# JARVIS-MoCap/JARVIS-HybridNet

Hardware: AMD Instinct MI355X
Metric: multi-view frames/s (12cam 1280x1024, 23kpt, 64^3 grid) (higher is better)
Workload: dtype f32; 1 GPU; BASELINE configs[2]: HybridNet 12-camera 1280x1024, 23 kpts, 64^3 grid, small/small; cameras=12, joints=23, grid=64, streams=3, parallelism=single GPU, 3 time batches in flight on 3 HIP streams, hipgraph=False

## Files before the change

### include/jarvis_hip.h

```cpp
#ifndef JARVIS_HIP_H
#define JARVIS_HIP_H
#include <stdint.h>

#ifdef __cplusplus
extern "C" {
#endif

#define JH_ABI_VERSION 4

const char* jh_last_error(void);
int jh_abi_version(void);

#define JH_PRECISION_DEFAULT (-1)
#define JH_PRECISION_F32 0
#define JH_PRECISION_BF16X3 1
#define JH_PRECISION_BF16X3_WIDE 2
int jh_set_precision(int mode);
int jh_get_precision(void);

typedef struct jh_params jh_params;
int jh_params_create(jh_params** out);
int jh_params_set(jh_params* p, const char* key, const float* host, int64_t numel);
void jh_params_destroy(jh_params* p);

typedef struct jh_efftrack jh_efftrack;
int jh_efftrack_create(const jh_params* p, const char* prefix, int model_size, int joints, int n,
                       int h, int w, int want_res1, jh_efftrack** out);
int jh_efftrack_forward(jh_efftrack* net, const float* x_dev, float* res1_dev, float* res2_dev,
                        void* stream);
int64_t jh_efftrack_launches(const jh_efftrack* net);
void jh_efftrack_destroy(jh_efftrack* net);

typedef struct jh_v2v jh_v2v;
int jh_v2v_create(const jh_params* p, const char* prefix, int joints, int t, int g, jh_v2v** out);
int jh_v2v_forward(jh_v2v* net, const float* x_dev, float* y_dev, void* stream);
void jh_v2v_destroy(jh_v2v* net);
int jh_v2v_fold(int joints, int t, int g, int* folded);

int64_t jh_reproject_workspace_bytes(int cams, int joints, int hs, int grid_size);
int jh_reproject_forward(const float* heatmaps_padded_dev, int cams, int joints, int hs,
                         const int32_t* center3d_dev, const int32_t* center_hm_dev,
                         const float* cam_dev, const float* intr_dev, const float* dist_dev,
                         int grid_size, float grid_spacing, float* vol_dev, int32_t* idx_dev,
                         void* workspace_dev, int64_t workspace_bytes, void* stream);

int64_t jh_softargmax_workspace_bytes(int t, int joints, int gh);
int jh_softargmax(const float* v2v_out_dev, int t, int joints, int gh, float grid_spacing,
                  float roi_cube_size, const int32_t* center3d_dev, float* heatmap_final_dev,
                  float* points_dev, float* conf_dev, void* workspace_dev, int64_t workspace_bytes,
                  void* stream);

int jh_reproject_point(const float* points_dev, int npoints, int cams, const float* cam_dev,
                       const float* intr_dev, const float* dist_dev, float* uv_dev, void* stream);
int64_t jh_reconstruct_workspace_bytes(int cams);
int jh_reconstruct_point(const float* points2d_dev, const float* maxvals_dev, int cams,
                         const float* cam_dev, const float* intr_dev, const float* dist_dev,
                         float* point3d_dev, void* workspace_dev, int64_t workspace_bytes,
                         void* stream);

typedef struct jh_predictor jh_predictor;
typedef struct {
  int32_t num_cameras, num_joints;
  int32_t center_size;
  int32_t bbox;
  float roi_cube_size;
  float grid_spacing;
  int32_t center_model, kp_model;
  int32_t img_h, img_w;
  int32_t time_batch;
  int32_t time_batch_3d;
  int32_t cam_lo, cam_n;
  float mean[3], std[3];
  int32_t precision;
} jh_predictor_config;

int jh_predictor_create(const jh_params* center_params, const jh_params* hybrid_params,
                        const jh_predictor_config* cfg, jh_predictor** out);
void jh_predictor_destroy(jh_predictor* pr);
int64_t jh_predictor_launches(const jh_predictor* pr);
int64_t jh_predictor_device_bytes(const jh_predictor* pr);
int jh_predictor_precision(const jh_predictor* pr);

int jh_predictor_set_calibration(jh_predictor* pr, const float* cam_dev, const float* intr_dev,
                                 const float* dist_dev, void* stream);
int jh_predictor_set_calibration_frames(jh_predictor* pr, const float* cam_dev ,
                                        const float* intr_dev , const float* dist_dev ,
                                        void* stream);

int jh_predictor_set_centers(jh_predictor* pr, const float* centers_dev , void* stream);

// ... 195 lines not shown
```

### jarvis-hybridnet_amd/_native.py

```python
import ctypes
import math
import os
from typing import NamedTuple

import torch

_HERE = os.path.dirname(os.path.abspath(__file__))
LIB_PATH = os.environ.get("JH_LIBRARY_PATH") or os.path.join(_HERE, "libjarvis_hip.so")
_lib = None

c_void_p, c_int, c_float, c_int64 = ctypes.c_void_p, ctypes.c_int, ctypes.c_float, ctypes.c_int64
c_char_p = ctypes.c_char_p


class PredictorConfig(ctypes.Structure):
    _fields_ = [("num_cameras", ctypes.c_int32), ("num_joints", ctypes.c_int32),
                ("center_size", ctypes.c_int32), ("bbox", ctypes.c_int32),
                ("roi_cube_size", c_float), ("grid_spacing", c_float),
                ("center_model", ctypes.c_int32), ("kp_model", ctypes.c_int32),
                ("img_h", ctypes.c_int32), ("img_w", ctypes.c_int32),
                ("time_batch", ctypes.c_int32), ("time_batch_3d", ctypes.c_int32),
                ("cam_lo", ctypes.c_int32),
                ("cam_n", ctypes.c_int32), ("mean", c_float * 3), ("std", c_float * 3),
                ("precision", ctypes.c_int32)]
# ... 13 lines not shown
    _fields_ = [("image_stride", ctypes.c_int64), ("offset", ctypes.c_int64), ("pitch", ctypes.c_int64),
                ("pattern", ctypes.c_int32), ("reserved", ctypes.c_int32)]


assert ctypes.sizeof(SensorSurfaceStruct) == 32

class OpOperand(ctypes.Structure):
    _fields_ = [("in_sums_host", c_void_p), ("in_act", ctypes.c_int32), ("latency_class", ctypes.c_int32),
                ("want_stats", ctypes.c_int32), ("se_c", ctypes.c_int32), ("se_s", ctypes.c_int32),
                ("se_inv_hw", c_float), ("se_wr_host", c_void_p), ("se_br_host", c_void_p),
                ("se_we_host", c_void_p), ("se_be_host", c_void_p), ("se_pool_host", c_void_p)]


assert ctypes.sizeof(OpOperand) == 72

class SubjectsParamsStruct(ctypes.Structure):
    _fields_ = [("max_subjects", ctypes.c_int32), ("max_peaks", ctypes.c_int32), ("nms_radius", ctypes.c_int32),
                ("min_views", ctypes.c_int32), ("min_peak", c_float), ("max_error_px", c_float)]


assert ctypes.sizeof(SubjectsParamsStruct) == 24

ABI_VERSION = 4
assert ctypes.sizeof(PredictorConfig) == 84

_WORKSPACES = {}


def workspace(nbytes, device):
    key = (str(device), torch.cuda.current_stream(device).cuda_stream)
    bufs = _WORKSPACES.setdefault(key, [])
    if not bufs or bufs[-1].numel() < nbytes:
        bufs.append(torch.empty((max(int(nbytes), 256),), dtype=torch.uint8, device=device))
    return bufs[-1]


_SIGS = {
    "jh_last_error": (c_char_p, []),
    "jh_abi_version": (c_int, []),
    "jh_set_precision": (c_int, [c_int]),
    "jh_get_precision": (c_int, []),
    "jh_params_create": (c_int, [ctypes.POINTER(c_void_p)]),
    "jh_params_set": (c_int, [c_void_p, c_char_p, c_void_p, c_int64]),
    "jh_params_destroy": (None, [c_void_p]),
    "jh_efftrack_create": (c_int, [c_void_p, c_char_p, c_int, c_int, c_int, c_int, c_int, c_int,
                                   ctypes.POINTER(c_void_p)]),
    "jh_efftrack_forward": (c_int, [c_void_p, c_void_p, c_void_p, c_void_p, c_void_p]),
    "jh_efftrack_launches": (c_int64, [c_void_p]),
    "jh_efftrack_destroy": (None, [c_void_p]),
    "jh_v2v_create": (c_int, [c_void_p, c_char_p, c_int, c_int, c_int, ctypes.POINTER(c_void_p)]),
    "jh_v2v_forward": (c_int, [c_void_p, c_void_p, c_void_p, c_void_p]),
    "jh_v2v_destroy": (None, [c_void_p]),
    "jh_v2v_fold": (c_int, [c_int, c_int, c_int, ctypes.POINTER(c_int)]),
    "jh_reproject_workspace_bytes": (c_int64, [c_int, c_int, c_int, c_int]),
    "jh_reproject_forward": (c_int, [c_void_p, c_int, c_int, c_int, c_void_p, c_void_p, c_void_p,
                                     c_void_p, c_void_p, c_int, c_float, c_void_p, c_void_p,
                                     c_void_p, c_int64, c_void_p]),
    "jh_softargmax_workspace_bytes": (c_int64, [c_int, c_int, c_int]),
    "jh_softargmax": (c_int, [c_void_p, c_int, c_int, c_int, c_float, c_float, c_void_p, c_void_p,
                              c_void_p, c_void_p, c_void_p, c_int64, c_void_p]),
    "jh_softargmax_spread_workspace_bytes": (c_int64, [c_int, c_int, c_int]),
    "jh_softargmax_spread": (c_int, [c_void_p, c_int, c_int, c_int, c_float, c_float, c_void_p, c_void_p,
                                     c_void_p, c_void_p, c_void_p, c_void_p, c_void_p, c_void_p, c_int64, c_void_p]),
    "jh_predictor_set_spread": (c_int, [c_void_p, c_int]),
    "jh_predictor_get_spread": (c_int, [c_void_p, c_void_p, c_void_p, c_void_p, c_void_p]),
    "jh_predictor_debug_v2v": (c_int, [c_void_p, c_void_p, c_void_p]),
    "jh_reproject_point": (c_int, [c_void_p, c_int, c_int, c_void_p, c_void_p, c_void_p, c_void_p,
                                   c_void_p]),
    "jh_reconstruct_workspace_bytes": (c_int64, [c_int]),
    "jh_reconstruct_point": (c_int, [c_void_p, c_void_p, c_int, c_void_p, c_void_p, c_void_p,
                                     c_void_p, c_void_p, c_int64, c_void_p]),
    "jh_predictor_create": (c_int, [c_void_p, c_void_p, ctypes.POINTER(PredictorConfig),
                                    ctypes.POINTER(c_void_p)]),
    "jh_predictor_destroy": (None, [c_void_p]),
    "jh_predictor_set_graph_replay": (c_int, [c_void_p, c_int]),
    "jh_predictor_graph_replay": (c_int, [c_void_p]),
    "jh_predictor_launches": (c_int64, [c_void_p]),
    "jh_predictor_device_bytes": (c_int64, [c_void_p]),
    "jh_predictor_precision": (c_int, [c_void_p]),
    "jh_predictor_set_calibration": (c_int, [c_void_p, c_void_p, c_void_p, c_void_p, c_void_p]),
    "jh_predictor_set_calibration_frames": (c_int, [c_void_p, c_void_p, c_void_p, c_void_p, c_void_p]),
    "jh_predictor_set_centers": (c_int, [c_void_p, c_void_p, c_void_p]),
    "jh_predictor_stage_center": (c_int, [c_void_p, c_void_p, c_void_p, c_void_p]),
    "jh_predictor_stage_keypoints": (c_int, [c_void_p, c_void_p, c_void_p, c_void_p, c_void_p]),
    "jh_predictor_stage_3d": (c_int, [c_void_p, c_void_p, c_int, c_void_p, c_void_p, c_void_p,
                                      c_void_p]),
    "jh_predictor_stage_keypoints_gathered": (c_int, [c_void_p, c_void_p, c_int, c_void_p, c_int, c_void_p,
                                                      c_void_p]),
    "jh_predictor_stage_3d_blocks": (c_int, [c_void_p, c_void_p, c_int, c_int, c_int, c_int, c_void_p,
                                             c_void_p, c_void_p, c_void_p]),
    "jh_profile_begin": (c_int, []),
    "jh_profile_end": (c_int, [ctypes.POINTER(c_int)]),
    "jh_profile_get": (c_int, [c_int, c_char_p, c_int, ctypes.POINTER(ctypes.c_double),
                               ctypes.POINTER(ctypes.c_double), ctypes.POINTER(ctypes.c_double)]),
    "jh_predictor_forward": (c_int, [c_void_p, c_void_p, c_void_p, c_void_p, c_void_p, c_void_p]),
    "jh_predictor_stage_center_u8": (c_int, [c_void_p, c_void_p, c_void_p, c_void_p]),
    "jh_predictor_stage_keypoints_u8": (c_int, [c_void_p, c_void_p, c_void_p, c_void_p, c_void_p]),
    "jh_predictor_forward_u8": (c_int, [c_void_p, c_void_p, c_void_p, c_void_p, c_void_p, c_void_p]),
    "jh_predictor_forward_yuv": (c_int, [c_void_p, c_void_p, c_int, c_void_p, c_void_p, c_void_p, c_void_p]),
    "jh_yuv_surface_check": (c_int, [ctypes.POINTER(YuvSurfaceStruct), c_int, c_int]),
    "jh_predictor_forward_surface": (c_int, [c_void_p, c_void_p, ctypes.POINTER(YuvSurfaceStruct), c_void_p, c_void_p,
                                             c_void_p, c_void_p, c_void_p]),
    "jh_predictor2d_forward_surface": (c_int, [c_void_p, c_void_p, ctypes.POINTER(YuvSurfaceStruct), c_void_p,
                                               c_void_p, c_void_p, c_void_p]),
    "jh_op_yuv_surface_to_bgr": (c_int, [c_void_p, ctypes.POINTER(YuvSurfaceStruct), c_int, c_int, c_int, c_void_p,
                                         c_void_p]),
# ... 404 lines not shown
```

### jarvis-hybridnet_amd/csrc/api.hip

```cpp
#include <cstring>
#include <memory>
#include "../../include/jarvis_hip.h"
#include <cstdlib>
#include "nets.h"
#include "bifpn_node.h"
#include "views2d.h"
#include "subjects.h"

namespace jh {
static thread_local std::string g_err;
void set_error(const std::string& msg) { g_err = msg; }
}

using namespace jh;

struct jh_params { ParamMap map; };
struct jh_efftrack { EffTrackPlan plan; };
struct jh_v2v { V2VPlan plan; };

namespace {

struct Scratch {
  std::vector<void*> ptrs;
  ~Scratch() { for (void* p : ptrs) (void)hipFree(p); }
// ... 126 lines not shown
  return 0;
}
int jh_get_precision(void) { return precision_mode(); }

int jh_params_create(jh_params** out) {
  *out = new jh_params();
  return 0;
}
int jh_params_set(jh_params* p, const char* key, const float* host, int64_t numel) {
  JH_REQUIRE(p && key && host && numel >= 0, "bad argument");
  p->map[key] = std::vector<float>(host, host + numel);
  return 0;
}
void jh_params_destroy(jh_params* p) { delete p; }

int jh_efftrack_create(const jh_params* p, const char* prefix, int model_size, int joints, int n,
                       int h, int w, int want_res1, jh_efftrack** out) {
  JH_REQUIRE(p && out, "bad argument");
  std::unique_ptr<jh_efftrack> net(new jh_efftrack());
  if (net->plan.build(p->map, prefix ? prefix : "", model_size, joints, n, h, w, want_res1 != 0)) return 1;
  *out = net.release();
  return 0;
}
int jh_efftrack_forward(jh_efftrack* net, const float* x_dev, float* res1_dev, float* res2_dev,
                        void* stream) {
  hipStream_t s = static_cast<hipStream_t>(stream);
  JH_REQUIRE(net && x_dev && res2_dev, "bad argument");
  JH_REQUIRE(!res1_dev || net->plan.res1.p, "res1 requested from a network created with want_res1 = 0");
  if (launch_to_channel_last(x_dev, net->plan.input, s)) return 1;
  if (net->plan.run(s)) return 1;
  if (res1_dev && launch_from_channel_last(net->plan.res1, res1_dev, s)) return 1;
  return launch_from_channel_last(net->plan.heat, res2_dev, s);
}
int64_t jh_efftrack_launches(const jh_efftrack* net) { return (int64_t)net->plan.launches(); }
void jh_efftrack_destroy(jh_efftrack* net) { delete net; }

int jh_v2v_create(const jh_params* p, const char* prefix, int joints, int t, int g, jh_v2v** out) {
  JH_REQUIRE(p && out, "bad argument");
  std::unique_ptr<jh_v2v> net(new jh_v2v());
  if (net->plan.build(p->map, prefix ? prefix : "", joints, t, g)) return 1;
  *out = net.release();
  return 0;
}
int jh_v2v_forward(jh_v2v* net, const float* x_dev, float* y_dev, void* stream) {
  hipStream_t s = static_cast<hipStream_t>(stream);
  if (launch_to_channel_last(x_dev, net->plan.input, s)) return 1;
  if (net->plan.run(s)) return 1;
  return launch_from_channel_last(net->plan.output, y_dev, s);
}
void jh_v2v_destroy(jh_v2v* net) { delete net; }
int jh_v2v_fold(int joints, int t, int g, int* folded) {
  JH_REQUIRE(joints >= 1 && t >= 1 && g >= 4 && g % 4 == 0 && folded, "jh_v2v_fold: bad argument");
  *folded = v2v_fold_applies(joints, g) ? 1 : 0;
  return 0;
}

int64_t jh_reproject_workspace_bytes(int cams, int joints, int hs, int grid_size) {
  Carver c(nullptr, 0);
  ReproWs w;
  return (int64_t)carve_reproject(c, cams, joints, hs, grid_size, &w);
}

int jh_reproject_forward(const float* heatmaps_padded_dev, int cams, int joints, int hs,
                         const int32_t* center3d_dev, const int32_t* center_hm_dev,
                         const float* cam_dev, const float* intr_dev, const float* dist_dev,
                         int grid_size, float grid_spacing, float* vol_dev, int32_t* idx_dev,
                         void* workspace_dev, int64_t workspace_bytes, void* stream) {
  hipStream_t s = static_cast<hipStream_t>(stream);
  JH_REQUIRE(workspace_dev && workspace_bytes >= 0, "workspace (see jh_reproject_workspace_bytes)");
  JH_REQUIRE(grid_size > 0 && grid_size % 2 == 0, "grid size must be even");
  Carver c(workspace_dev, (size_t)workspace_bytes);
  ReproWs w;
  carve_reproject(c, cams, joints, hs, grid_size, &w);
  JH_REQUIRE(c.fits(), "workspace smaller than jh_reproject_workspace_bytes()");
  if (launch_to_channel_last(heatmaps_padded_dev, w.heat, s)) return 1;
  if (launch_reproject(Calib{cam_dev, intr_dev, dist_dev, 0}, center3d_dev, center_hm_dev, w.heat.p, w.coarse,
                       w.vol.p, idx_dev, 1, cams, grid_size, grid_spacing, hs, w.heat.Cp,
                       1, 0, nullptr, s)) return 1;
  return launch_from_channel_last(w.vol, vol_dev, s);
}

int64_t jh_softargmax_workspace_bytes(int t, int joints, int gh) {
  Carver c(nullptr, 0);
  SoftWs w;
  return (int64_t)carve_softargmax(c, t, joints, gh, &w);
}

int jh_softargmax(const float* v2v_out_dev, int t, int joints, int gh, float grid_spacing,
                  float roi_cube_size, const int32_t* center3d_dev, float* heatmap_final_dev,
                  float* points_dev, float* conf_dev, void* workspace_dev, int64_t workspace_bytes,
                  void* stream) {
  hipStream_t s = static_cast<hipStream_t>(stream);
  JH_REQUIRE(workspace_dev && workspace_bytes >= 0, "workspace (see jh_softargmax_workspace_bytes)");
  Carver c(workspace_dev, (size_t)workspace_bytes);
  SoftWs w;
  carve_softargmax(c, t, joints, gh, &w);
  JH_REQUIRE(c.fits(), "workspace smaller than jh_softargmax_workspace_bytes()");
  if (launch_to_channel_last(v2v_out_dev, w.x, s)) return 1;
  return launch_softargmax(w.x.p, center3d_dev, w.partial, w.pmax, points_dev, conf_dev,
                           heatmap_final_dev, t, joints, w.x.Cp, gh, grid_spacing, roi_cube_size, s);
}

int64_t jh_softargmax_spread_workspace_bytes(int t, int joints, int gh) {
  Carver c(nullptr, 0);
  SoftWs w;
  SoftargmaxSpread sp;
// ... 1463 lines not shown
```

### jarvis-hybridnet_amd/csrc/conv_host.hip

```cpp
#include <vector>
#include <cstring>
#include <algorithm>
#include "conv_mfma.h"

namespace jh {

ConvDesc conv_desc(int nd, int k, int stride, int pad, int cin, int cout) {
  ConvDesc d{};
  d.nd = nd; d.k = k; d.stride = stride; d.ostride = 1; d.nphase = 1;
  d.cin = cin; d.cout = cout;
  d.phase[0].pad[0] = (nd == 3) ? pad : 0;
  d.phase[0].pad[1] = pad; d.phase[0].pad[2] = pad;
  d.phase[0].ooff[0] = d.phase[0].ooff[1] = d.phase[0].ooff[2] = 0;
  return d;
}

ConvDesc deconv2d_k4s2p1_desc(int cin, int cout) {
  ConvDesc d{};
  d.nd = 2; d.k = 2; d.stride = 1; d.ostride = 2; d.nphase = 4;
  d.cin = cin; d.cout = cout;
  for (int py = 0; py < 2; ++py)
    for (int px = 0; px < 2; ++px) {
      ConvPhase& p = d.phase[py * 2 + px];
      p.pad[0] = 0; p.pad[1] = py ? 0 : 1; p.pad[2] = px ? 0 : 1;
// ... 67 lines not shown
              const int nbk = co / 16, nn = co % 16;
              const int lane = kq * 16 + nn;
              if (tap_paired)
                packed[((((size_t)(tap / 2)) * nk8 + kc8) * nb + nbk) * 256 + lane * 4 + (tap & 1) * 2 + j] = v;
              else if (window) {
                const int sub = (1 - d.phase[ph].ooff[1]) * 2 + (1 - d.phase[ph].ooff[2]);
                const int col = sub * cout_p + co;
                packed[(((size_t)tap * npair + kc8 / 2) * nbw + col / 16) * 256 + (kq * 16 + col % 16) * 4 +
                       (kc8 & 1) * 2 + j] = v;
              }
              else if (paired)
                packed[ph * phase_stride + (((size_t)tap * (nk8 / 2) + kc8 / 2) * nb + nbk) * 256 + lane * 4 + (kc8 & 1) * 2 + j] = v;
              else
                packed[ph * phase_stride + (((size_t)tap * nk8 + kc8) * nb + nbk) * 128 + lane * 2 + j] = v;
            }
        }
  }
  out->cin_p = cin_p; out->cout_p16 = cout_p16; out->layout = layout;
  out->phase_stride = tap_paired ? packed.size() : (window ? packed.size() / d.nphase : phase_stride);
  return upload_conv_weights(packed.data(), packed.size() * sizeof(float), b, d.cout, out);
}

int upload_conv_weights(const void* packed, size_t bytes, const float* b, int cout, ConvWeights* out) {
  out->bias = nullptr;
  JH_CHECK_HIP(hipMalloc(reinterpret_cast<void**>(&out->w), bytes));
  JH_CHECK_HIP(hipMemcpy(out->w, packed, bytes, hipMemcpyHostToDevice));
  if (!b) return 0;
  std::vector<float> bp(out->cout_p16, 0.f);
  std::memcpy(bp.data(), b, cout * sizeof(float));
  JH_CHECK_HIP(hipMalloc(&out->bias, bp.size() * sizeof(float)));
  JH_CHECK_HIP(hipMemcpy(out->bias, bp.data(), bp.size() * sizeof(float), hipMemcpyHostToDevice));
  return 0;
}

void free_conv_weights(ConvWeights* w) {
  if (w->w) (void)hipFree(w->w);
  if (w->bias) (void)hipFree(w->bias);
  w->w = w->bias = nullptr;
}

static int pick_nr(int nb, int taps, bool heavy_staging, long units) {
  const double stage = (heavy_staging ? 1.5 : 0.5) / (double)taps;
  const long slots = 512;
  int best = 1;
  double best_cost = 1e30;
  for (int nr = 4; nr >= 1; --nr) {
    const long groups = (nb + nr - 1) / nr;
    const double cost = (double)std::max(units * groups, slots) * (stage + nr);
    if (cost < best_cost - 1e-9) { best_cost = cost; best = nr; }
  }
  return best;
}

int launch_conv(const ConvDesc& d, const ConvWeights& w, const Act& x, const Act& y,
                const float* gate, double* stats, hipStream_t s, const InNorm* in, const SeGate* se) {
  JH_REQUIRE(x.Cp == w.cin_p || (x.Cp == 4 && w.cin_p == 8), "conv input channel padding mismatch");
  JH_REQUIRE(y.Cp == cpad(d.cout), "conv output channel padding mismatch");
  JH_REQUIRE(x.N == y.N, "batch mismatch");
  ConvArgs a{};
  a.x = x.p; a.y = y.p; a.w = w.w; a.bias = w.bias; a.gate = gate; a.stats = stats;
  if (in && in->stats) {
    a.in_stats = in->stats; a.in_inv = in->inv; a.in_act = in->act;
    a.nrm_floats = 2 * w.cin_p;
  }
  if (gate) a.nrm_floats += w.cin_p;
  if (se && se->pool) {
    JH_REQUIRE(!gate, "either a gate tensor or a gate recipe");
    a.se = *se;
    a.nrm_floats += w.cin_p + round_up(se->C, 4) + round_up(se->S, 4);
  }
  a.N = x.N; a.Din = x.D; a.Hin = x.H; a.Win = x.W; a.cin_p = w.cin_p; a.in_px = x.Cp;
  a.Dy = y.D; a.Hy = y.H; a.Wy = y.W; a.cout_p = y.Cp; a.cout_p16 = w.cout_p16;
  a.ostride = d.ostride; a.nphase = d.nphase; a.phase_stride = w.phase_stride; a.layout = w.layout;
  for (int p = 0; p < d.nphase; ++p) a.phase[p] = d.phase[p];
  if (d.ostride > 1) { a.Dout = x.D; a.Hout = x.H; a.Wout = x.W; }
  else conv_out_shape(d, x.D, x.H, x.W, &a.Dout, &a.Hout, &a.Wout);
  int Do, Ho, Wo;
  conv_out_shape(d, x.D, x.H, x.W, &Do, &Ho, &Wo);
  JH_REQUIRE(Do == y.D && Ho == y.H && Wo == y.W, "conv output extent mismatch");
  const int taps = d.k * d.k * (d.nd == 3 ? d.k : 1);
  long units;
  if (d.nd == 2) units = (long)((a.Hout + 7) / 8) * ((a.Wout <= 8 ? a.Wout + 7 : a.Wout + 15) / (a.Wout <= 8 ? 8 : 16));
  else units = (long)((a.Dout + 1) / 2) * ((a.Hout + 3) / 4) * ((a.Wout + 15) / 16);
  units *= (long)a.nphase * a.N;
  const int nr = pick_nr(w.cout_p16 / 16, taps, (in && in->stats && in->act == ACT_SILU) || gate || (se && se->pool),
                         units);
  const size_t budget = kConvLdsBudget;
  switch (w.layout) {
    case WeightLayout::Window: return launch_deconv4_window(a, s);
    case WeightLayout::ChannelPaired: return launch_deconv4_fused(a, s);
    case WeightLayout::TapPaired: case WeightLayout::Plain: break;
  }
  if (conv_pw_direct_eligible(d, a)) return launch_conv_pw_direct(a, s);
  if (d.nd == 2) {
    const int small = (a.Wout <= 8) ? 1 : 0;
    const int big = (a.Wout >= 64 && a.Hout >= 64 && w.cin_p <= 32 && d.ostride == 1 && d.stride == 1 &&
               (d.k == 1 || d.k == 3)) ? 1 : 0;
    if (big) return conv_launch_2d_big(a, d.k, d.stride, nr, budget, s);
    if (d.k == 1 && d.stride == 1 && d.ostride == 1 && d.nphase == 1 && (a.Wout % 16 != 0 || a.Hout % 8 != 0) &&
        a.Hout * a.Wout >= 96 && a.Hin == a.Hout && a.Win == a.Wout && a.Hy == a.Hout && a.Wy == a.Wout) {
      ConvArgs f = a;
      f.Win = f.Wout = f.Wy = a.Hout * a.Wout;
      f.Hin = f.Hout = f.Hy = 1;
      return conv_launch_2d_k1_flat(f, nr, budget, s);
    }
    if (d.k == 1 && d.stride == 1) return conv_launch_2d_k1(a, nr, small, budget, s);
    if (d.k == 2 && d.stride == 1) return conv_launch_2d_k2(a, nr, small, budget, s);
    if (d.k == 3 && d.stride == 1 && d.ostride == 1 && a.Wout > 16 && a.Wout <= 20 && a.Hout <= 22 &&
        !d.latency_class)
      return conv_launch_2d_k3_w20(a, nr, std::max(budget, (size_t)64 * 1024), s);
    if (!d.latency_class && d.ostride == 1) {
      if (d.k == 5 && d.stride <= 2 && a.Wout > 32 && a.Wout <= 40)
        return conv_launch_2d_k5_w40(a, d.stride, nr, std::max(budget, (size_t)64 * 1024), s);
      if (d.k == 3 && d.stride == 2 && a.Wout > 16 && a.Wout <= 20 && a.Hout <= 22)
        return conv_launch_2d_k3s2_w20(a, nr, std::max(budget, (size_t)96 * 1024), s);
    }
    if (d.k == 3 && d.stride <= 2) return conv_launch_2d_k3(a, d.stride, nr, small, budget, s);
    if (d.k == 5 && d.stride <= 2) return conv_launch_2d_k5(a, d.stride, nr, small, budget, s);
  } else {
    const int nr_form = pick_nr(w.cout_p16 / 16, taps,
                                (in && in->stats && in->act == ACT_SILU) || gate || (se && se->pool), 1L << 40);
    const long tiles_big = (long)((a.Dout + 1) / 2) * ((a.Hout + 3) / 4) * ((a.Wout + 15) / 16) *
                           a.nphase * ((w.cout_p16 / 16 + nr_form - 1) / nr_form);
    int small = tiles_big < 16 ? 1 : 0;
    if (!small && d.k == 3 && d.stride == 1 && tiles_big >= 256) small = 2;
    if (d.k == 1 && d.stride == 1) return conv_launch_3d_k1(a, nr, small, budget, s);
    if (d.k == 2 && d.stride == 2) return conv_launch_3d_k2s2(a, nr, small, budget, s);
    if (d.k == 3 && d.stride <= 2) return conv_launch_3d_k3(a, d.stride, nr, small, budget, s);
  }
  JH_REQUIRE(false, "no convolution kernel for this (nd, k, stride)");
}

}
```

### jarvis-hybridnet_amd/csrc/jh_common.h

```cpp
#pragma once
#include <hip/hip_runtime.h>
#include <cstdlib>
#include <cstdint>
#include <cstdio>
#include <cstring>
#include <string>
#include <vector>

namespace jh {

constexpr int kWave = 64;

#define JH_ENV_KNOB(name) ([]() -> int { static const int v = [] { const char* e = getenv(name); return e ? atoi(e) : -1; }(); return v; }())

inline int round_up(int v, int m) { return (v + m - 1) / m * m; }
inline int cpad(int c) { return round_up(c, 8); }

void set_error(const std::string& msg);
#define JH_CHECK_HIP(expr)                                                     \
  do {                                                                         \
    hipError_t _e = (expr);                                                    \
    if (_e != hipSuccess) {                                                    \
      jh::set_error(std::string(#expr) + ": " + hipGetErrorString(_e));        \
      return 1;                                                                \
// ... 214 lines not shown
  const unsigned L = blockIdx.x + gx * (blockIdx.y + gy * blockIdx.z);
  const unsigned l = xcd_linear(L, gx * gy * gz);
  BlockId b;
  const unsigned l1 = fd_div(l, fgx);
  b.x = l - l1 * gx;
  b.z = fd_div(l1, fgy);
  b.y = l1 - b.z * gy;
  return b;
}
__device__ __forceinline__ BlockId xcd_block() {
  const unsigned gx = gridDim.x, gy = gridDim.y, gz = gridDim.z;
  const unsigned L = blockIdx.x + gx * (blockIdx.y + gy * blockIdx.z);
  unsigned l = xcd_linear(L, gx * gy * gz);
  BlockId b;
  b.x = l % gx; l /= gx;
  b.y = l % gy;
  b.z = l / gy;
  return b;
}
#endif

#if defined(__HIPCC__)
__device__ __forceinline__ float sum_xor16(float s) {
  const auto r = __builtin_amdgcn_permlane16_swap(__float_as_uint(s), __float_as_uint(s), false, false);
  return __uint_as_float(r[0]) + __uint_as_float(r[1]);
}
__device__ __forceinline__ float sum_xor32(float s) {
  const auto r = __builtin_amdgcn_permlane32_swap(__float_as_uint(s), __float_as_uint(s), false, false);
  return __uint_as_float(r[0]) + __uint_as_float(r[1]);
}
__device__ __forceinline__ double sum_xor16(double s) {
  const unsigned lo = (unsigned)__double2loint(s), hi = (unsigned)__double2hiint(s);
  const auto a = __builtin_amdgcn_permlane16_swap(lo, lo, false, false);
  const auto b = __builtin_amdgcn_permlane16_swap(hi, hi, false, false);
  return __hiloint2double((int)b[0], (int)a[0]) + __hiloint2double((int)b[1], (int)a[1]);
}
__device__ __forceinline__ double sum_xor32(double s) {
  const unsigned lo = (unsigned)__double2loint(s), hi = (unsigned)__double2hiint(s);
  const auto a = __builtin_amdgcn_permlane32_swap(lo, lo, false, false);
  const auto b = __builtin_amdgcn_permlane32_swap(hi, hi, false, false);
  return __hiloint2double((int)b[0], (int)a[0]) + __hiloint2double((int)b[1], (int)a[1]);
}
__device__ __forceinline__ float silu_fast(float v) { return v * __builtin_amdgcn_rcpf(1.f + __expf(-v)); }
#endif

int pack_wino_weights(int cin, int cout, const float* w, const float* b, ConvWeights* out);
int launch_conv3d_wino(const ConvWeights& w, const Act& x, const Act& y, double* stats, hipStream_t s,
                       const InNorm* in, int variant, const int* tables);
bool v2v_fold_shape(int J, int G);
bool v2v_fold_applies(int J, int G);
int launch_conv3d_out_fold(const ConvWeights& w, const Act& r_dec, const double* st_dec, const float* u0,
                           const double* st_u0, const float* r_skip, const double* st_skip, const float* f1,
                           const Act& y, hipStream_t s);
inline unsigned short bf16_rne(float f) {
  unsigned u;
  std::memcpy(&u, &f, 4);
  u += 0x7fffu + ((u >> 16) & 1u);
  return (unsigned short)(u >> 16);
}
inline float bf16_to_f32(unsigned short h) {
  const unsigned u = (unsigned)h << 16;
  float f;
  std::memcpy(&f, &u, 4);
  return f;
}
int pack_bf16x3_weights(int cin, int cout, const float* w, const float* b, ConvWeights* out);
int launch_conv3d_bf16x3(const ConvWeights& w, const Act& x, const Act& y, double* stats, hipStream_t s,
                         const InNorm* in);
int pack_deconv4_bf16x3_weights(int cin, int cout, const float* w, ConvWeights* out);
bool deconv4_bf16x3_eligible(int cout);
int launch_deconv4_bf16x3(const ConvWeights& w, const Act& x, const Act& y, hipStream_t s, const InNorm* in);
bool conv_bf16x3_eligible(const ConvDesc& d);
int pack_conv_bf16x3_weights(const ConvDesc& d, const float* w, const float* b, ConvWeights* out);
int launch_conv_bf16x3(const ConvDesc& d, const ConvWeights& w, const Act& x, const Act& y, double* stats,
                       hipStream_t s, const InNorm* in);
int precision_mode();
void set_precision_mode(int m);
void pack_stem_weights(const float* w_host, float* packed, int cout);
int launch_stem_conv(const Act& x, const float* w_dev, const Act& y, double* stats, hipStream_t s);
struct StemSource;
int launch_stem_conv_src(const StemSource& src, const Act& x, const float* w_dev, const Act& y, double* stats,
                         hipStream_t s);
int launch_deconv_c1(const Act& x, const double* stats, float inv_cnt, int in_act, const float* w,
                     const Act& y, hipStream_t s);

int launch_zero(void* p, size_t bytes, hipStream_t s);

int launch_to_channel_last(const float* src, const Act& dst, hipStream_t s);
int launch_from_channel_last(const Act& src, float* dst, hipStream_t s);

}
```

### jarvis-hybridnet_amd/csrc/nets.hip

```cpp
#include <cmath>
#include <cstring>
#include <cstdlib>
#include "nets.h"
#include "bifpn_node.h"

namespace jh {

Profiler& profiler() {
  static Profiler p;
  return p;
}
void Profiler::begin(const std::string& name, double flops, double bytes, hipStream_t s) {
  ProfRec r{name, flops, bytes, nullptr, nullptr, 0.f};
  (void)hipEventCreate(&r.e0);
  (void)hipEventCreate(&r.e1);
  (void)hipEventRecord(r.e0, s);
  recs.push_back(r);
}
void Profiler::end(hipStream_t s) { (void)hipEventRecord(recs.back().e1, s); }
int Profiler::finish() {
  JH_CHECK_HIP(hipDeviceSynchronize());
  for (auto& r : recs) {
    if (!r.e0) continue;
    JH_CHECK_HIP(hipEventElapsedTime(&r.ms, r.e0, r.e1));
// ... 445 lines not shown
        const Ref in[2] = {p7_in, p6_out};
        if (fnode("p7_w2", 2, in, m_dn2, p7_in, "conv7_down", &p7_out)) return 1;
      }
    }
    p3 = p3_out; p4 = p4_out; p5 = p5_out; p6 = p6_out; p7 = p7_out;
  }

  const float* wc = nullptr;
  if (get(pm, pre + "weights_cat", 3, &wc)) return 1;
  float w[3], sum = 0.f;
  for (int i = 0; i < 3; ++i) { w[i] = wc[i] > 20.f ? wc[i] : log1pf(expf(wc[i])); sum += w[i]; }
  for (int i = 0; i < 3; ++i) w[i] = w[i] / (sum + 0.0001f);
  const Ref hin[3] = {p3, p4, p5};
  const int hmodes[3] = {FUSE_SAME, FUSE_UP2, FUSE_UP4};
  Ref mid;
  if (node(pm, pre + "first_conv.", 3, hin, hmodes, w, ACT_NONE, p3.a, ss.head, &mid)) return 1;
  if (new_act(N, 1, mid.a.H * 2, mid.a.W * 2, J, &heat)) return 1;
  if (want_res1) {
    if (new_act(N, 1, mid.a.H, mid.a.W, J, &res1)) return 1;
    if (add_conv(pm, conv_desc(2, 3, 1, 1, ss.head, J), pre + "final_conv1.weight", "", false, mid.a,
                 res1, nullptr, false, nullptr, mid.st, mid.inv, ACT_NONE)) return 1;
  }
  if (add_conv(pm, deconv2d_k4s2p1_desc(ss.head, J), pre + "deconv1.weight", "", true, mid.a, heat,
               nullptr, false, nullptr, mid.st, mid.inv, ACT_NONE)) return 1;
  return finish();
}

int V2VPlan::res_block(const ParamMap& pm, const std::string& p, int c, const Act& x,
                       const float* extra, Act* out, long x_stats, size_t* raw_stats) {
  Act a;
  if (new_act(x.N, x.D, x.H, x.W, c, &a)) return 1;
  size_t s1 = 0, s2 = 0;
  const float inv = 1.f / (float)(x.D * x.H * x.W);
  if (add_conv(pm, conv_desc(3, 3, 1, 1, c, c), p + "res_branch.0.weight", p + "res_branch.0.bias",
               false, x, a, nullptr, true, &s1, x_stats, inv, ACT_RELU)) return 1;
  if (new_act(x.N, x.D, x.H, x.W, c, out)) return 1;
  if (add_conv(pm, conv_desc(3, 3, 1, 1, c, c), p + "res_branch.3.weight", p + "res_branch.3.bias",
               false, a, *out, nullptr, true, &s2, (long)s1, 1.f / (float)(x.D * x.H * x.W),
               ACT_RELU)) return 1;
  if (raw_stats) { *raw_stats = s2; return 0; }
  add_norm(*out, s2, ACT_RELU, x.p, extra, out->p, -1, x_stats);
  return 0;
}

int V2VPlan::build(const ParamMap& pm, const std::string& pre, int J, int T, int G) {
  JH_REQUIRE(G % 4 == 0, "grid size must be a multiple of 4");
  const int Gh = G / 2, Gq = G / 4;
  if (new_act(T, G, G, G, J, &input)) return 1;
  Act f0, f1, skip, e0, e1, u0, d1;
  size_t st = 0;
  if (new_act(T, Gh, Gh, Gh, 2 * J, &f0)) return 1;
  if (add_conv(pm, conv_desc(3, 3, 2, 1, J, 2 * J), pre + "front_layers.0.block.0.weight",
               pre + "front_layers.0.block.0.bias", false, input, f0, nullptr, true, &st)) return 1;
  if (res_block(pm, pre + "front_layers.1.", 2 * J, f0, nullptr, &f1, (long)st)) return 1;
  const std::string e = pre + "encoder_decoder.";
  const bool fold = v2v_fold_applies(J, G);
  size_t st_skip = 0, st_dec = 0;
  if (res_block(pm, e + "skip_res1.", 2 * J, f1, nullptr, &skip, -1, fold ? &st_skip : nullptr)) return 1;
  if (new_act(T, Gq, Gq, Gq, 4 * J, &e0)) return 1;
  if (add_conv(pm, conv_desc(3, 2, 2, 0, 2 * J, 4 * J), e + "encoder_pool1.block.0.weight",
               e + "encoder_pool1.block.0.bias", false, f1, e0, nullptr, true, &st)) return 1;
  if (res_block(pm, e + "mid_res.", 4 * J, e0, nullptr, &e1, (long)st)) return 1;
  if (new_act(T, Gh, Gh, Gh, 2 * J, &u0)) return 1;
  if (add_conv(pm, deconv3d_k2s2_desc(4 * J, 2 * J), e + "decoder_upsample1.block.0.weight",
               e + "decoder_upsample1.block.0.bias", true, e1, u0, nullptr, true, &st)) return 1;
  const size_t st_u0 = st;
  if (res_block(pm, e + "decoder_res1.", 2 * J, u0, skip.p, &d1, (long)st, fold ? &st_dec : nullptr)) return 1;
  if (new_act(T, Gh, Gh, Gh, J, &output)) return 1;
  if (!fold) {
    if (add_conv(pm, conv_desc(3, 1, 1, 0, 2 * J, J), pre + "output_layer.weight",
                 pre + "output_layer.bias", false, d1, output, nullptr, false, nullptr)) return 1;
    return finish();
  }
  const float *w = nullptr, *b = nullptr;
  if (get(pm, pre + "output_layer.weight", (size_t)2 * J * J, &w)) return 1;
  if (get(pm, pre + "output_layer.bias", J, &b)) return 1;
  ConvUse use;
  use.desc = conv_desc(3, 1, 1, 0, 2 * J, J);
  use.has_bias = true; use.precision = precision; use.in_px = d1.Cp;
  layers_.emplace_back();
  const ConvLayer* layer = &layers_.back();
  if (make_conv_layer(use, w, b, Gh, Gh, Gh, &layers_.back())) return 1;
  JH_REQUIRE(layer->choice.form == ConvForm::Mfma && layer->choice.layout == WeightLayout::Plain,
             "output fold: the 1 x 1 x 1 layer's weight layout");
  bytes_ += layer->device_bytes();
  const double vox = (double)T * d1.pixels();
  char nm[96];
  snprintf(nm, sizeof nm, "conv3d_k1s1fold_%dx%d@%d", 2 * J, J, Gh);
  push(nm, 2.0 * vox * 2 * J * J, 4.0 * (vox * (4.0 * d1.Cp + output.Cp) + 2.0 * J * J),
       [this, layer, d1, u0, skip, f1, st_dec, st_u0, st_skip](hipStream_t s) {
    return launch_conv3d_out_fold(layer->w, d1, sc(st_dec), u0.p, sc(st_u0), skip.p, sc(st_skip), f1.p, output, s);
  });
  return finish();
}

}
```

Before: 2203 multi-view frames/s.

## Fuse mid_res block closing norm/residual/ReLU into the k2s2 upsample deconv

Adds a dedicated MFMA kernel that applies the mid residual block's final instance norm, residual add with the normalized encoder input, and ReLU while loading operands for the transposed k2s2 upsample conv. The separate normalization pass that wrote e1 to memory and the extra read are dropped, cutting one kernel launch and a full activation round trip. It adds a new specialized kernel with fixed template instances and weight prefetching. It is gated by an env var that defaults on, and only applies to supported joint counts and grid sizes.

```diff
diff --git a/include/jarvis_hip.h b/include/jarvis_hip.h
--- a/include/jarvis_hip.h
+++ b/include/jarvis_hip.h
@@ -36,6 +36,7 @@
 int jh_v2v_forward(jh_v2v* net, const float* x_dev, float* y_dev, void* stream);
 void jh_v2v_destroy(jh_v2v* net);
 int jh_v2v_fold(int joints, int t, int g, int* folded);
+int jh_v2v_close(int joints, int t, int g, int* closed);
 
 int64_t jh_reproject_workspace_bytes(int cams, int joints, int hs, int grid_size);
 int jh_reproject_forward(const float* heatmaps_padded_dev, int cams, int joints, int hs,
diff --git a/jarvis-hybridnet_amd/_native.py b/jarvis-hybridnet_amd/_native.py
--- a/jarvis-hybridnet_amd/_native.py
+++ b/jarvis-hybridnet_amd/_native.py
@@ -89,6 +89,7 @@
     "jh_v2v_forward": (c_int, [c_void_p, c_void_p, c_void_p, c_void_p]),
     "jh_v2v_destroy": (None, [c_void_p]),
     "jh_v2v_fold": (c_int, [c_int, c_int, c_int, ctypes.POINTER(c_int)]),
+    "jh_v2v_close": (c_int, [c_int, c_int, c_int, ctypes.POINTER(c_int)]),
     "jh_reproject_workspace_bytes": (c_int64, [c_int, c_int, c_int, c_int]),
     "jh_reproject_forward": (c_int, [c_void_p, c_int, c_int, c_int, c_void_p, c_void_p, c_void_p,
                                      c_void_p, c_void_p, c_int, c_float, c_void_p, c_void_p,
diff --git a/jarvis-hybridnet_amd/csrc/api.hip b/jarvis-hybridnet_amd/csrc/api.hip
--- a/jarvis-hybridnet_amd/csrc/api.hip
+++ b/jarvis-hybridnet_amd/csrc/api.hip
@@ -202,6 +202,11 @@
 int jh_v2v_fold(int joints, int t, int g, int* folded) {
   JH_REQUIRE(joints >= 1 && t >= 1 && g >= 4 && g % 4 == 0 && folded, "jh_v2v_fold: bad argument");
   *folded = v2v_fold_applies(joints, g) ? 1 : 0;
+  return 0;
+}
+int jh_v2v_close(int joints, int t, int g, int* closed) {
+  JH_REQUIRE(joints >= 1 && t >= 1 && g >= 4 && g % 4 == 0 && closed, "jh_v2v_close: bad argument");
+  *closed = v2v_close_applies(joints, g) ? 1 : 0;
   return 0;
 }
 
diff --git a/jarvis-hybridnet_amd/csrc/conv3d_close.hip b/jarvis-hybridnet_amd/csrc/conv3d_close.hip
--- /dev/null
+++ b/jarvis-hybridnet_amd/csrc/conv3d_close.hip
@@ -0,0 +1,216 @@
+#include "conv_mfma.h"
+
+namespace jh {
+
+namespace {
+typedef float cf4 __attribute__((ext_vector_type(4)));
+typedef unsigned cu4 __attribute__((ext_vector_type(4)));
+typedef unsigned cu2 __attribute__((ext_vector_type(2)));
+
+struct CloseArgs {
+  const float *r, *x0;
+  const double *st_r, *st_x0;
+  const float *w, *bias;
+  float* f1;
+  float* y;
+  double* stats;
+  int D, H, W, Cp;
+  int cout_p, cout_p16;
+  int phase_stride;
+};
+
+__device__ __forceinline__ void close_coefs(const CloseArgs& a, int n, int P, float (*nrm)[2][128], int tid) {
+  for (int i = tid; i < 2 * a.Cp; i += 256) {
+    const int slot = i >= a.Cp ? 1 : 0, c = i - slot * a.Cp;
+    const NormCoef k = norm_coef_over_count((slot ? a.st_x0 : a.st_r) + ((size_t)n * a.Cp + c) * kStatW, P);
+    nrm[slot][0][c] = k.mean;
+    nrm[slot][1][c] = k.rstd;
+  }
+  __syncthreads();
+}
+
+__device__ __forceinline__ cf4 close4(cf4 r, cf4 x0, cf4 mu_r, cf4 rs_r, cf4 mu_x, cf4 rs_x) {
+  cf4 t = (r - mu_r) * rs_r;
+  cf4 e = (x0 - mu_x) * rs_x;
+#pragma unroll
+  for (int i = 0; i < 4; ++i) e[i] = fmaxf(e[i], 0.f);
+  t += e;
+#pragma unroll
+  for (int i = 0; i < 4; ++i) t[i] = fmaxf(t[i], 0.f);
+  return t;
+}
+
+__device__ __forceinline__ void to_operands(cf4 v, float2& s0, float2& s1) {
+  const auto x0 = __builtin_amdgcn_permlane16_swap(__float_as_uint(v[0]), __float_as_uint(v[2]), false, false);
+  const auto x1 = __builtin_amdgcn_permlane16_swap(__float_as_uint(v[1]), __float_as_uint(v[3]), false, false);
+  const auto z0 = __builtin_amdgcn_permlane32_swap(x0[0], x0[1], false, false);
+  const auto z1 = __builtin_amdgcn_permlane32_swap(x1[0], x1[1], false, false);
+  s0 = make_float2(__uint_as_float(z0[0]), __uint_as_float(z1[0]));
+  s1 = make_float2(__uint_as_float(z0[1]), __uint_as_float(z1[1]));
+}
+
+template <int K8, int NCB>
+__global__ __launch_bounds__(256, 2) void conv3d_close_up_kernel(const CloseArgs a, int nph) {
+  constexpr int KW = (K8 + 1) / 2;
+  __shared__ __attribute__((aligned(16))) float nrm_s[2][2][128];
+  __shared__ __attribute__((aligned(16))) double red_s[4 * NCB * 16 * 2];
+  const int tid = threadIdx.x;
+  const int lane = tid & 63;
+  const int wave = __builtin_amdgcn_readfirstlane(tid >> 6);
+  const int px = lane & 15, kq = lane >> 4;
+  const int n = blockIdx.z;
+  const int Cp = a.Cp;
+  const int P = a.D * a.H * a.W;
+  close_coefs(a, n, P, nrm_s, tid);
+
+  const int tiles_x = a.W >> 4, tiles_y = a.H >> 2;
+  const int tile_x = blockIdx.x % tiles_x, t1 = blockIdx.x / tiles_x;
+  const int tile_y = t1 % tiles_y, tile_z = t1 / tiles_y;
+  const int oz0 = tile_z * 2, oy0 = tile_y * 4, ox0 = tile_x * 16;
+
+  const size_t img = (size_t)n * P * Cp;
+  const int img_bytes = (int)((size_t)P * Cp * 4);
+  const __amdgpu_buffer_rsrc_t rs_r = __builtin_amdgcn_make_buffer_rsrc(const_cast<float*>(a.r + img), 0, img_bytes, 0x00020000);
+  const __amdgpu_buffer_rsrc_t rs_x = __builtin_amdgcn_make_buffer_rsrc(const_cast<float*>(a.x0 + img), 0, img_bytes, 0x00020000);
+
+  float2 av[2][2 * KW];
+#pragma unroll
+  for (int mr = 0; mr < 2; ++mr) {
+    const int rb = wave * 2 + mr;
+    const int vox = ((oz0 + (rb >> 2)) * a.H + oy0 + (rb & 3)) * a.W + ox0 + px;
+    cf4 r[KW], x[KW];
+#pragma unroll
+    for (int u = 0; u < KW; ++u) {
+      const int off = 16 * u + 4 * kq < Cp ? (vox * Cp + 16 * u + 4 * kq) * 4 : (int)0x80000000;
+      r[u] = __builtin_bit_cast(cf4, __builtin_amdgcn_raw_buffer_load_b128(rs_r, off, 0, 0));
+      x[u] = __builtin_bit_cast(cf4, __builtin_amdgcn_raw_buffer_load_b128(rs_x, off, 0, 0));
+    }
+#pragma unroll
+    for (int u = 0; u < KW; ++u) {
+      const bool in = 16 * u + 4 * kq < Cp;
+      cf4 m[2], s[2];
+#pragma unroll
+      for (int sl = 0; sl < 2; ++sl) {
+        m[sl] = in ? *reinterpret_cast<const cf4*>(&nrm_s[sl][0][16 * u + 4 * kq]) : (cf4){0.f, 0.f, 0.f, 0.f};
+        s[sl] = in ? *reinterpret_cast<const cf4*>(&nrm_s[sl][1][16 * u + 4 * kq]) : (cf4){1.f, 1.f, 1.f, 1.f};
+      }
+      to_operands(close4(r[u], x[u], m[0], s[0], m[1], s[1]), av[mr][2 * u], av[mr][2 * u + 1]);
+    }
+  }
+
+  EpilogueArgs e;
+  e.y = a.y + (size_t)n * 8 * P * a.cout_p;
+  e.bias = a.bias;
+  e.stats = a.stats + (size_t)n * a.cout_p * kStatW;
+  e.Dout = a.D; e.Hout = a.H; e.Wout = a.W; e.Hy = 2 * a.H; e.Wy = 2 * a.W;
+  e.cout_p = a.cout_p; e.cout_p16 = a.cout_p16; e.os = 2; e.osz = 2;
+
+  const int ph0 = blockIdx.y * nph;
+  const __amdgpu_buffer_rsrc_t wrs = __builtin_amdgcn_make_buffer_rsrc(
+      const_cast<float*>(a.w), 0, 7 * a.phase_stride * 4 + K8 * NCB * 128 * 4, 0x00020000);
+  constexpr int PD = 2;
+  static_assert(K8 >= PD, "the prefetch distance");
+  float2 b[PD + 1][NCB], bnext[PD][NCB];
+  auto wload = [&](int ph, int k8, float2 (&dst)[NCB]) __attribute__((always_inline)) {
+#pragma unroll
+    for (int cb = 0; cb < NCB; ++cb) {
+      const cu2 v = __builtin_amdgcn_raw_buffer_load_b64(wrs, lane * 8, ph * a.phase_stride * 4 + (k8 * NCB + cb) * 512, 0);
+      dst[cb] = make_float2(__uint_as_float(v.x), __uint_as_float(v.y));
+    }
+  };
+#pragma unroll
+  for (int k8 = 0; k8 < PD; ++k8) wload(ph0, k8, bnext[k8]);
+  for (int ph = ph0; ph < ph0 + nph; ++ph) {
+    const int phn = min(ph + 1, ph0 + nph - 1);
+    f32x4 acc[2][NCB];
+#pragma unroll
+    for (int mr = 0; mr < 2; ++mr)
+#pragma unroll
+      for (int cb = 0; cb < NCB; ++cb) acc[mr][cb] = (f32x4){0.f, 0.f, 0.f, 0.f};
+#pragma unroll
+    for (int k8 = 0; k8 < PD; ++k8)
+#pragma unroll
+      for (int cb = 0; cb < NCB; ++cb) b[k8][cb] = bnext[k8][cb];
+#pragma unroll
+    for (int k8 = 0; k8 < K8; ++k8) {
+      if (k8 + PD < K8) wload(ph, k8 + PD, b[(k8 + PD) % (PD + 1)]);
+      else wload(phn, k8 + PD - K8, bnext[k8 + PD - K8]);
+#pragma unroll
+      for (int mr = 0; mr < 2; ++mr)
+#pragma unroll
+        for (int cb = 0; cb < NCB; ++cb)
+          acc[mr][cb] = __builtin_amdgcn_mfma_f32_16x16x4f32(av[mr][k8].x, b[k8 % (PD + 1)][cb].x, acc[mr][cb], 0, 0, 0);
+#pragma unroll
+      for (int mr = 0; mr < 2; ++mr)
+#pragma unroll
+        for (int cb = 0; cb < NCB; ++cb)
+          acc[mr][cb] = __builtin_amdgcn_mfma_f32_16x16x4f32(av[mr][k8].y, b[k8 % (PD + 1)][cb].y, acc[mr][cb], 0, 0, 0);
+      __builtin_amdgcn_sched_barrier(0);
+    }
+    e.offz = (ph >> 2) & 1; e.offy = (ph >> 1) & 1; e.offx = ph & 1;
+    __syncthreads();
+    conv_epilogue<2, NCB, 4, 16, 4, true>(acc, e, reinterpret_cast<float*>(red_s), 0, oz0, oy0, ox0, tid);
+  }
+}
+
+struct CloseInst { int k8a, ncba, k8b, ncbb; };
+constexpr CloseInst kCloseInst[] = {{2, 2, 3, 1}, {6, 6, 12, 3}, {8, 8, 15, 4}};
+
+int close_inst(int J) {
+  const CloseInst want = {cpad(2 * J) / 8, round_up(4 * J, 16) / 16, cpad(4 * J) / 8, round_up(2 * J, 16) / 16};
+  for (int i = 0; i < (int)(sizeof kCloseInst / sizeof kCloseInst[0]); ++i)
+    if (kCloseInst[i].k8a == want.k8a && kCloseInst[i].ncba == want.ncba && kCloseInst[i].k8b == want.k8b &&
+        kCloseInst[i].ncbb == want.ncbb)
+      return i;
+  return -1;
+}
+}
+
+bool v2v_close_shape(int J, int G) {
+  return J >= 1 && G >= 64 && G % 64 == 0 && G <= 256 && close_inst(J) >= 0;
+}
+
+bool v2v_close_applies(int J, int G) {
+  const char* e = getenv("JH_V2V_CLOSE");
+  return (e ? atoi(e) : 1) != 0 && v2v_close_shape(J, G);
+}
+
+static int close_args(const ConvWeights& w, const Act& r, const double* st_r, const float* x0, const double* st_x0,
+                      const Act& y, double* st_y, CloseArgs* a) {
+  JH_REQUIRE(w.layout == WeightLayout::Plain && w.cin_p == r.Cp && w.cout_p16 == round_up(y.C, 16) && w.bias,
+             "close: the packed weights of the layer");
+  JH_REQUIRE(y.N == r.N && y.Cp == cpad(y.C) && st_r && x0 && st_x0 && st_y, "close: operands");
+  JH_REQUIRE(r.Cp <= 128 && r.pixels() * r.Cp * 4 < ((size_t)1 << 31) && y.pixels() * y.Cp * 4 < ((size_t)1 << 31),
+             "close: shape (v2v_close_shape)");
+  a->r = r.p; a->x0 = x0; a->st_r = st_r; a->st_x0 = st_x0;
+  a->w = w.w; a->bias = w.bias; a->f1 = nullptr; a->y = y.p; a->stats = st_y;
+  a->D = r.D; a->H = r.H; a->W = r.W; a->Cp = r.Cp;
+  a->cout_p = y.Cp; a->cout_p16 = w.cout_p16; a->phase_stride = (int)w.phase_stride;
+  return 0;
+}
+
+int launch_conv3d_close_up(const ConvDesc& d, const ConvWeights& w, const Act& r, const double* st_r, const float* e0,
+                           const double* st_e0, const Act& u0, double* st_u0, hipStream_t s) {
+  CloseArgs a;
+  if (close_args(w, r, st_r, e0, st_e0, u0, st_u0, &a)) return 1;
+  JH_REQUIRE(u0.D == 2 * r.D && u0.H == 2 * r.H && u0.W == 2 * r.W && r.D % 2 == 0 && r.H % 4 == 0 && r.W % 16 == 0,
+             "close + upsample: whole 2 x 4 x 16 tiles (v2v_close_shape)");
+  JH_REQUIRE(d.nphase == 8 && conv3d_tile_class(d, w.cout_p16, false, r.D, r.H, r.W) == 0,
+             "close + upsample: the layer's tile on the general path is 2 x 4 x 16");
+  const int k8 = a.Cp / 8, ncb = w.cout_p16 / 16;
+  const int tiles = (r.D / 2) * (r.H / 4) * (r.W / 16);
+  int nph = 8;
+  while (nph > 1 && (long)tiles * r.N * (8 / nph) < 512) nph >>= 1;
+  const dim3 grid(tiles, 8 / nph, r.N);
+#define JH_CU(K8V, NCBV)                                                                                          \
+  if (k8 == K8V && ncb == NCBV) {                                                                                 \
+    hipLaunchKernelGGL((conv3d_close_up_kernel<K8V, NCBV>), grid, dim3(256), 0, s, a, nph);                       \
+    JH_CHECK_HIP(hipGetLastError());                                                                              \
+    return 0;                                                                                                     \
+  }
+  JH_CU(3, 1) JH_CU(12, 3) JH_CU(15, 4)
+#undef JH_CU
+  JH_REQUIRE(false, "close + upsample: no kernel for this channel count");
+}
+
+}
diff --git a/jarvis-hybridnet_amd/csrc/conv_host.hip b/jarvis-hybridnet_amd/csrc/conv_host.hip
--- a/jarvis-hybridnet_amd/csrc/conv_host.hip
+++ b/jarvis-hybridnet_amd/csrc/conv_host.hip
@@ -143,6 +143,16 @@
   return best;
 }
 
+int conv3d_tile_class(const ConvDesc& d, int cout_p16, bool heavy_staging, int Dout, int Hout, int Wout) {
+  const int taps = d.k * d.k * (d.nd == 3 ? d.k : 1);
+  const int nr_form = pick_nr(cout_p16 / 16, taps, heavy_staging, 1L << 40);
+  const long tiles_big = (long)((Dout + 1) / 2) * ((Hout + 3) / 4) * ((Wout + 15) / 16) *
+                         d.nphase * ((cout_p16 / 16 + nr_form - 1) / nr_form);
+  int small = tiles_big < 16 ? 1 : 0;
+  if (!small && d.k == 3 && d.stride == 1 && tiles_big >= 256) small = 2;
+  return small;
+}
+
 int launch_conv(const ConvDesc& d, const ConvWeights& w, const Act& x, const Act& y,
                 const float* gate, double* stats, hipStream_t s, const InNorm* in, const SeGate* se) {
   JH_REQUIRE(x.Cp == w.cin_p || (x.Cp == 4 && w.cin_p == 8), "conv input channel padding mismatch");
@@ -209,12 +219,8 @@
     if (d.k == 3 && d.stride <= 2) return conv_launch_2d_k3(a, d.stride, nr, small, budget, s);
     if (d.k == 5 && d.stride <= 2) return conv_launch_2d_k5(a, d.stride, nr, small, budget, s);
   } else {
-    const int nr_form = pick_nr(w.cout_p16 / 16, taps,
-                                (in && in->stats && in->act == ACT_SILU) || gate || (se && se->pool), 1L << 40);
-    const long tiles_big = (long)((a.Dout + 1) / 2) * ((a.Hout + 3) / 4) * ((a.Wout + 15) / 16) *
-                           a.nphase * ((w.cout_p16 / 16 + nr_form - 1) / nr_form);
-    int small = tiles_big < 16 ? 1 : 0;
-    if (!small && d.k == 3 && d.stride == 1 && tiles_big >= 256) small = 2;
+    const int small = conv3d_tile_class(d, w.cout_p16, (in && in->stats && in->act == ACT_SILU) || gate || (se && se->pool),
+                                        a.Dout, a.Hout, a.Wout);
     if (d.k == 1 && d.stride == 1) return conv_launch_3d_k1(a, nr, small, budget, s);
     if (d.k == 2 && d.stride == 2) return conv_launch_3d_k2s2(a, nr, small, budget, s);
     if (d.k == 3 && d.stride <= 2) return conv_launch_3d_k3(a, d.stride, nr, small, budget, s);
diff --git a/jarvis-hybridnet_amd/csrc/jh_common.h b/jarvis-hybridnet_amd/csrc/jh_common.h
--- a/jarvis-hybridnet_amd/csrc/jh_common.h
+++ b/jarvis-hybridnet_amd/csrc/jh_common.h
@@ -290,6 +290,11 @@
 int launch_conv3d_out_fold(const ConvWeights& w, const Act& r_dec, const double* st_dec, const float* u0,
                            const double* st_u0, const float* r_skip, const double* st_skip, const float* f1,
                            const Act& y, hipStream_t s);
+bool v2v_close_shape(int J, int G);
+bool v2v_close_applies(int J, int G);
+int launch_conv3d_close_up(const ConvDesc& d, const ConvWeights& w, const Act& r, const double* st_r, const float* e0,
+                           const double* st_e0, const Act& u0, double* st_u0, hipStream_t s);
+int conv3d_tile_class(const ConvDesc& d, int cout_p16, bool heavy_staging, int Dout, int Hout, int Wout);
 inline unsigned short bf16_rne(float f) {
   unsigned u;
   std::memcpy(&u, &f, 4);
diff --git a/jarvis-hybridnet_amd/csrc/nets.hip b/jarvis-hybridnet_amd/csrc/nets.hip
--- a/jarvis-hybridnet_amd/csrc/nets.hip
+++ b/jarvis-hybridnet_amd/csrc/nets.hip
@@ -521,6 +521,24 @@
   if (new_act(T, Gh, Gh, Gh, 2 * J, &f0)) return 1;
   if (add_conv(pm, conv_desc(3, 3, 2, 1, J, 2 * J), pre + "front_layers.0.block.0.weight",
                pre + "front_layers.0.block.0.bias", false, input, f0, nullptr, true, &st)) return 1;
+  const bool close = v2v_close_applies(J, G);
+  auto close_layer = [&](const ConvDesc& d, const std::string& key, bool transposed, int in_px, int Dy,
+                         const ConvLayer** out) -> int {
+    const float *w = nullptr, *b = nullptr;
+    if (get(pm, key + "weight", (size_t)d.cin * d.cout * 8, &w)) return 1;
+    if (get(pm, key + "bias", d.cout, &b)) return 1;
+    ConvUse use;
+    use.desc = d; use.desc.latency_class = norm_block_kb == 0 ? 1 : 0;
+    use.transposed = transposed; use.has_bias = true; use.want_stats = true; use.precision = precision;
+    use.in_px = in_px;
+    layers_.emplace_back();
+    *out = &layers_.back();
+    if (make_conv_layer(use, w, b, Dy, Dy, Dy, &layers_.back())) return 1;
+    JH_REQUIRE((*out)->choice.form == ConvForm::Mfma && (*out)->choice.layout == WeightLayout::Plain,
+               "close: the k2 s2 layer's weight layout");
+    bytes_ += (*out)->device_bytes();
+    return 0;
+  };
   if (res_block(pm, pre + "front_layers.1.", 2 * J, f0, nullptr, &f1, (long)st)) return 1;
   const std::string e = pre + "encoder_decoder.";
   const bool fold = v2v_fold_applies(J, G);
@@ -529,10 +547,26 @@
   if (new_act(T, Gq, Gq, Gq, 4 * J, &e0)) return 1;
   if (add_conv(pm, conv_desc(3, 2, 2, 0, 2 * J, 4 * J), e + "encoder_pool1.block.0.weight",
                e + "encoder_pool1.block.0.bias", false, f1, e0, nullptr, true, &st)) return 1;
-  if (res_block(pm, e + "mid_res.", 4 * J, e0, nullptr, &e1, (long)st)) return 1;
+  const size_t st_e0 = st;
+  size_t st_rm = 0;
+  if (res_block(pm, e + "mid_res.", 4 * J, e0, nullptr, &e1, (long)st, close ? &st_rm : nullptr)) return 1;
   if (new_act(T, Gh, Gh, Gh, 2 * J, &u0)) return 1;
-  if (add_conv(pm, deconv3d_k2s2_desc(4 * J, 2 * J), e + "decoder_upsample1.block.0.weight",
-               e + "decoder_upsample1.block.0.bias", true, e1, u0, nullptr, true, &st)) return 1;
+  if (!close) {
+    if (add_conv(pm, deconv3d_k2s2_desc(4 * J, 2 * J), e + "decoder_upsample1.block.0.weight",
+                 e + "decoder_upsample1.block.0.bias", true, e1, u0, nullptr, true, &st)) return 1;
+  } else {
+    const ConvLayer* layer = nullptr;
+    if (close_layer(deconv3d_k2s2_desc(4 * J, 2 * J), e + "decoder_upsample1.block.0.", true, e1.Cp, Gh, &layer)) return 1;
+    st = scratch((size_t)T * u0.Cp * kStatW);
+    const size_t st_up = st;
+    const double vox = (double)T * e1.pixels();
+    char nm[96];
+    snprintf(nm, sizeof nm, "conv3d_k2s2Tclose_%dx%d@%d", 4 * J, 2 * J, Gh);
+    push(nm, 2.0 * vox * 8 * 4 * J * 2 * J, 4.0 * (vox * (2.0 * e1.Cp + 8.0 * u0.Cp) + 8.0 * 4 * J * 2 * J),
+         [this, layer, e1, e0, u0, st_rm, st_e0, st_up](hipStream_t s) {
+      return launch_conv3d_close_up(layer->desc, layer->w, e1, sc(st_rm), e0.p, sc(st_e0), u0, sc(st_up), s);
+    });
+  }
   const size_t st_u0 = st;
   if (res_block(pm, e + "decoder_res1.", 2 * J, u0, skip.p, &d1, (long)st, fold ? &st_dec : nullptr)) return 1;
   if (new_act(T, Gh, Gh, Gh, J, &output)) return 1;
```

Result: no change. 2202 multi-view frames/s (-0.0%).
